# jontio/JAERO

Measured on NVIDIA H100. Metric: IQ Msamples/s (10.5k OQPSK demod + Viterbi), higher is better.
Workload: dtype f64

## Files before the change

jaero_b200/csrc/capi.cu:

```cuda
#include "../../include/jaero_b200.h"
#include "common.cuh"
#include "viterbi.cuh"
#include "demod.cuh"
#include "prefilter.cuh"
#include "pchannel.cuh"
#include "burst.cuh"
#include "rtchannel.cuh"
#include "cchannel.cuh"
#include "ddc.cuh"
#include "scan.cuh"
#include <cstring>
#include <complex>
#include <climits>
#include <cstdlib>
#include <initializer_list>
#include <new>
#include <numeric>
#include <vector>

namespace jb {
static thread_local std::string g_err;
void set_error(const std::string &m) { g_err = m; }
int cuda_fail(cudaError_t e, const char *what, const char *file, int line)
{
// ... 671 lines not shown
        b->slot_of.resize(cp);
        std::vector<int> ident(cp);
        for (size_t c = 0; c < cp; c++) { ident[c] = (int)c; b->slot_of[c] = (int)c; }
        JB_CUDA(cudaMemcpy(b->d_chan_of, ident.data(), cp * sizeof(int), cudaMemcpyHostToDevice));
        p.chan_of = b->d_chan_of;
        b->next_regroup = 34;
    }
    JB_CUDA(cudaMallocHost(&b->h_ints, (size_t)I_COUNT * cp * sizeof(int)));
    JB_CUDA(cudaMallocHost(&b->h_dbls, (size_t)D_COUNT * cp * sizeof(double)));
    JB_CUDA(cudaMallocHost(&b->h_soft_total, cp * sizeof(long long)));
    JB_CUDA(cudaMallocHost(&b->h_soft_stage, (size_t)n_channels * p.soft_cap * sizeof(int16_t)));
    guard.release();
    *out = b;
    return JAERO_OK;
}

void jaero_batch_destroy(jaero_batch *b)
{
    if (!b) return;
    cudaSetDevice(b->device);
    cudaStreamSynchronize(b->stream);
    if (b->copy_stream) { cudaStreamSynchronize(b->copy_stream); cudaStreamDestroy(b->copy_stream); }
    if (b->ev_stage_free) cudaEventDestroy(b->ev_stage_free);
    for (int k = 0; k < 8; k++) if (b->ev_slice[k]) cudaEventDestroy(b->ev_slice[k]);
    for (auto &e : b->ev_seg) { cudaEventDestroy(e.first); cudaEventDestroy(e.second); }
    for (auto &e : b->ev_cfe) { cudaEventDestroy(e.first); cudaEventDestroy(e.second); }
    release(b, {b->d_stage, b->d_x, b->d_ring_scratch}, {b->h_ints, b->h_dbls, b->h_soft_stage, b->h_soft_total, b->h_keys}, b->own_stream);
}
int jaero_batch_channels(const jaero_batch *b) { return b ? b->p.n_channels : 0; }
int64_t jaero_batch_launch_count(const jaero_batch *b) { return b ? b->launches : 0; }

int jaero_batch_set_stream(jaero_batch *b, void *cuda_stream)
{
    if (!b) { set_error("null handle"); return JAERO_E_ARG; }
    JB_CUDA(cudaSetDevice(b->device));
    JB_CUDA(cudaStreamSynchronize(b->stream));
    b->stream = cuda_stream ? (cudaStream_t)cuda_stream : b->own_stream;
    return JAERO_OK;
}
int jaero_batch_set_profiling(jaero_batch *b, int enabled)
{
    if (!b) { set_error("null handle"); return JAERO_E_ARG; }
    b->profiling = enabled != 0;
    return JAERO_OK;
}
int jaero_batch_get_profile(jaero_batch *b, double out[5])
{
    if (!b || !out) { set_error("null argument"); return JAERO_E_ARG; }
    JB_CUDA(cudaSetDevice(b->device));
    JB_CUDA(cudaStreamSynchronize(b->stream));
    double seg = 0, cfe = 0;
    for (auto &e : b->ev_seg) { float ms = 0; cudaEventElapsedTime(&ms, e.first, e.second); seg += ms; cudaEventDestroy(e.first); cudaEventDestroy(e.second); }
    for (auto &e : b->ev_cfe) { float ms = 0; cudaEventElapsedTime(&ms, e.first, e.second); cfe += ms; cudaEventDestroy(e.first); cudaEventDestroy(e.second); }
    out[0] = seg; out[1] = (double)b->ev_seg.size(); out[2] = cfe; out[3] = (double)b->ev_cfe.size(); out[4] = b->prof_samples;
    b->ev_seg.clear(); b->ev_cfe.clear(); b->prof_samples = 0;
    return JAERO_OK;
}
int jaero_batch_cfe_clusters(const jaero_batch *b) { return b ? b->cfe.clusters : 0; }

int jaero_batch_cfe_geometry(const jaero_batch *b, int32_t out[6])
{
    if (!b || !out) { set_error("jaero_batch_cfe_geometry: null argument"); return JAERO_E_ARG; }
    const CfePlan &c = b->cfe;
    out[0] = c.nfft; out[1] = b->p.bb_len; out[2] = c.lo; out[3] = c.hi; out[4] = c.expectedpeakbin; out[5] = c.clusters;
    return JAERO_OK;
}
int jaero_batch_probe_cfe(jaero_batch *b, const double *ring, int oldest, const int32_t *bigchange, int impl, int max_clusters,
                          int max_group, double *y_out, double *raw_est, double *emitted_est)
{
    if (!b || !ring) { set_error("jaero_batch_probe_cfe: null argument"); return JAERO_E_ARG; }
    DemodParams &p = b->p;
    const int C = p.n_channels, N = b->cfe.nfft;
    const size_t cp = p.cpad;
    if (oldest < 0 || oldest >= p.bb_len) { set_error("jaero_batch_probe_cfe: oldest outside the ring"); return JAERO_E_ARG; }
    if (impl < 0 || impl > 2 || max_clusters < 0 || max_group < 0) {
        set_error("jaero_batch_probe_cfe: bad impl / max_clusters / max_group"); return JAERO_E_ARG; }
    CfePlan plan = b->cfe;
    if (max_group > 0) plan.group = std::min(plan.group, max_group);
    JB_CUDA(cudaSetDevice(b->device));
    int clusters = b->cfe.clusters;
    if (impl == 1) clusters = 0;
    if (impl == 2) {
        clusters = (N == 16384) ? cfe_cluster_capacity() : 0;
        if (clusters <= 0) { set_error("jaero_batch_probe_cfe: the cluster estimator is not available for this batch / device"); return JAERO_E_STATE; }
    }
    if (clusters > 0 && max_clusters > 0) clusters = std::min(clusters, max_clusters);
    JB_CUDA(cudaStreamSynchronize(b->stream));
    const cudaStream_t s = b->stream;
    std::vector<int> em, zb;
    JB_CUDA(cudaMemcpyAsync(p.bb, ring, (size_t)C * p.bb_len * sizeof(double2), cudaMemcpyHostToDevice, s));
    if (bigchange) {
        em.resize(C); zb.resize(C);
        JB_CUDA(cudaMemcpyAsync(em.data(), p.I + (size_t)I_EMPTYING * cp, C * sizeof(int), cudaMemcpyDeviceToHost, s));
        JB_CUDA(cudaMemcpyAsync(zb.data(), p.I + (size_t)I_ZERO_BB * cp, C * sizeof(int), cudaMemcpyDeviceToHost, s));
        JB_CUDA(cudaStreamSynchronize(s));
        for (int c = 0; c < C; c++) if (bigchange[c]) { em[c] = 4; zb[c] = 1; }
        JB_CUDA(cudaMemcpyAsync(p.I + (size_t)I_EMPTYING * cp, em.data(), C * sizeof(int), cudaMemcpyHostToDevice, s));
        JB_CUDA(cudaMemcpyAsync(p.I + (size_t)I_ZERO_BB * cp, zb.data(), C * sizeof(int), cudaMemcpyHostToDevice, s));
    }
    if (clusters > 0 ? cfe_cluster_run(plan, p, oldest, std::min(clusters, C), s, &b->launches)
                     : cfe_run(plan, p, oldest, s, &b->launches)) return JAERO_E_CUDA;
    if (y_out) JB_CUDA(cudaMemcpyAsync(y_out, b->cfe.y, (size_t)C * N * sizeof(double), cudaMemcpyDeviceToHost, s));
    if (raw_est) JB_CUDA(cudaMemcpyAsync(raw_est, p.D + (size_t)D_CFE_EST * cp, C * sizeof(double), cudaMemcpyDeviceToHost, s));
    if (emitted_est) JB_CUDA(cudaMemcpyAsync(emitted_est, p.cfe_est_out, C * sizeof(double), cudaMemcpyDeviceToHost, s));
    JB_CUDA(cudaStreamSynchronize(s));
    return JAERO_OK;
}

int jaero_batch_sync(jaero_batch *b)
{
    if (!b) { set_error("null handle"); return JAERO_E_ARG; }
    JB_CUDA(cudaSetDevice(b->device));
    JB_CUDA(cudaStreamSynchronize(b->stream));
    return JAERO_OK;
}

int jaero_batch_write_device(jaero_batch *b, const int16_t *d_pcm, size_t n, size_t stride)
{
    if (!b || !d_pcm) { set_error("jaero_batch_write_device: null argument"); return JAERO_E_ARG; }
    if (n == 0) return JAERO_OK;
    if (stride < n || n > 0x7fffffff) { set_error("jaero_batch_write_device: bad stride / length"); return JAERO_E_ARG; }
    JB_CUDA(cudaSetDevice(b->device));
    const DemodParams &p = b->p;
    if ((((uintptr_t)d_pcm) & 15) || (stride & 7)) {
        const size_t C = p.n_channels, pitch = (n + 7) & ~(size_t)7;
        if (d_pcm == b->d_stage) { set_error("internal: staging buffer misaligned"); return JAERO_E_STATE; }
        if (grow(&b->d_stage, &b->stage_cap, C * pitch, b->stream)) return JAERO_E_CUDA;
        JB_CUDA(cudaMemcpy2DAsync(b->d_stage, pitch * sizeof(int16_t), d_pcm, stride * sizeof(int16_t), n * sizeof(int16_t), C,
                                  cudaMemcpyDeviceToDevice, b->stream));
        d_pcm = b->d_stage; stride = pitch;
    }
    if (b->pre_on) {
        while (b->next_slice < b->n_slices) { JB_CUDA(cudaStreamWaitEvent(b->stream, b->ev_slice[b->next_slice], 0)); b->next_slice++; }
        const size_t C = p.n_channels, xs = (n + 7) & ~(size_t)7;
        if (grow(&b->d_x, &b->x_cap, C * xs, b->stream)) return JAERO_E_CUDA;
        b->pre.x = b->d_x; b->pre.xstride = xs;
        b->p.xpre = b->d_x; b->p.xstride = xs;
        if (pre_down_launch(b->pre, d_pcm, stride, (int)n, b->stream)) return JAERO_E_CUDA;
        b->launches++;
        int i = 0;
        while (i < (int)n) {
            const int room = FIR_L - b->fir_fill;
            const int take = std::min(room, (int)n - i);
            if (fir_exchange_up_launch(b->pre, b->fir, i, i + take, b->fir_fill, b->stream)) return JAERO_E_CUDA;
            b->launches++;
            b->fir_fill += take; i += take;
            if (b->fir_fill == FIR_L) {
                if (fir_block_launch(b->fir, p.n_channels, b->fir_blocks == 0 ? 1 : 0, b->stream)) return JAERO_E_CUDA;
                b->launches++;
                b->fir_fill = 0; b->fir_blocks++;
            }
        }
    }
    peak_kernel<<<(p.n_channels + 3) / 4, 128, 0, b->stream>>>(p, d_pcm, stride, (int)n);
    JB_CUDA(cudaGetLastError());
    b->launches++;
    const int N = p.bbnfft, trig_every = p.cpu_reduce ? N : N / 4;
    SegmentArgs a;
    memset(&a, 0, sizeof a);
    a.new_write = 1;
    int seg_start = 0; bool resume = false;
    auto launch = [&](int i0, int i1, bool stop_after_a, int bb0, int cc0) -> int {
        a.sample0 = b->samples; a.i0 = i0; a.i1 = i1; a.skip_a_first = resume ? 1 : 0; a.stop_after_a = stop_after_a ? 1 : 0;
        a.apply_cfe = resume ? 1 : 0; a.bb_pos = bb0; a.coarse_counter = cc0;
        while (b->next_slice < b->n_slices && b->next_slice * b->slice_len < i1) {
            JB_CUDA(cudaStreamWaitEvent(b->stream, b->ev_slice[b->next_slice], 0));
            b->next_slice++;
        }
        cudaEvent_t e0 = 0, e1 = 0;
        if (b->profiling) { cudaEventCreate(&e0); cudaEventCreate(&e1); cudaEventRecord(e0, b->stream); }
        int r = (p.kind == JAERO_KIND_MSK) ? msk_pipe_launch(p, a, d_pcm, stride, b->stream)
                : (p.fb > 8400)            ? oqpsk_pipe_launch(p, a, d_pcm, stride, b->stream)
                                           : oqpsk_segment_launch(p, a, d_pcm, stride, b->stream);
        if (b->profiling) { cudaEventRecord(e1, b->stream); b->ev_seg.push_back({e0, e1}); b->prof_samples += (i1 - i0 - (stop_after_a ? 1 : 0)); }
        b->launches++;
        a.new_write = 0;
        return r;
    };
    int bb = b->bb_pos, cc = b->coarse_counter;
    int seg_bb = bb, seg_cc = cc;
    for (int i = 0; i < (int)n; i++) {
        bool trigger = false;
        if (cc >= p.Fs || !p.cpu_reduce) {
            bb++; if (bb >= N) bb = 0;
            if (bb % trig_every == 0) trigger = true;
        }
        if (trigger) {
            if (launch(seg_start, i + 1, true, seg_bb, seg_cc)) return JAERO_E_CUDA;
            b->samples += (i - seg_start);
            cudaEvent_t c0 = 0, c1 = 0;
            if (b->profiling) { cudaEventCreate(&c0); cudaEventCreate(&c1); cudaEventRecord(c0, b->stream); }
            if (b->cfe.clusters > 0 ? cfe_cluster_run(b->cfe, p, bb, std::min(b->cfe.clusters, p.n_channels), b->stream, &b->launches)
                                    : cfe_run(b->cfe, p, bb, b->stream, &b->launches)) return JAERO_E_CUDA;
            if (b->profiling) { cudaEventRecord(c1, b->stream); b->ev_cfe.push_back({c0, c1}); }
            b->epochs++;
            if (b->next_regroup >= 0 && b->epochs >= b->next_regroup) {
                b->next_regroup = b->epochs + (b->epochs < 64 ? 32 : REGROUP_EVERY);
                if (batch_regroup_by_phase(b, false)) return JAERO_E_CUDA;
            }
            cc = 0;
            seg_start = i; resume = true; seg_bb = bb; seg_cc = 0;
        }
        cc++;
    }
    if (launch(seg_start, (int)n, false, seg_bb, seg_cc)) return JAERO_E_CUDA;
    b->samples += ((int)n - seg_start);
    while (b->next_slice < b->n_slices) { JB_CUDA(cudaStreamWaitEvent(b->stream, b->ev_slice[b->next_slice], 0)); b->next_slice++; }
    b->n_slices = 0; b->next_slice = 0;
    b->bb_pos = bb; b->coarse_counter = cc;
    if (b->pre_on) {
        if (pre_finish_launch(b->pre, p.m2_freq_sum, (int)n, p.Fs, b->stream)) return JAERO_E_CUDA;
        b->launches++;
    }
    return JAERO_OK;
}

int jaero_batch_write(jaero_batch *b, const int16_t *pcm, size_t n, size_t stride)
{
    if (!b || !pcm) { set_error("jaero_batch_write: null argument"); return JAERO_E_ARG; }
    if (n == 0) return JAERO_OK;
    if (stride < n) { set_error("jaero_batch_write: channel_stride < n_samples"); return JAERO_E_ARG; }
    JB_CUDA(cudaSetDevice(b->device));
    const size_t C = b->p.n_channels;
    const size_t pitch = (n + 7) & ~(size_t)7;
    if (grow(&b->d_stage, &b->stage_cap, C * pitch, b->stream)) return JAERO_E_CUDA;
    if (n < 8192) {
        JB_CUDA(cudaMemcpy2DAsync(b->d_stage, pitch * sizeof(int16_t), pcm, stride * sizeof(int16_t), n * sizeof(int16_t), C,
                                  cudaMemcpyHostToDevice, b->stream));
        return jaero_batch_write_device(b, b->d_stage, n, pitch);
    }
    if (!b->copy_stream) {
        JB_CUDA(cudaStreamCreateWithFlags(&b->copy_stream, cudaStreamNonBlocking));
        JB_CUDA(cudaEventCreateWithFlags(&b->ev_stage_free, cudaEventDisableTiming));
        for (int k = 0; k < 8; k++) JB_CUDA(cudaEventCreateWithFlags(&b->ev_slice[k], cudaEventDisableTiming));
    }
    JB_CUDA(cudaEventRecord(b->ev_stage_free, b->stream));
    JB_CUDA(cudaStreamWaitEvent(b->copy_stream, b->ev_stage_free, 0));
    b->slice_len = (int)((((n + 7) / 8) + 7) & ~(size_t)7);
    b->n_slices = 0; b->next_slice = 0;
    for (size_t s0 = 0; s0 < n; s0 += (size_t)b->slice_len) {
        const size_t len = std::min((size_t)b->slice_len, n - s0);
        JB_CUDA(cudaMemcpy2DAsync(b->d_stage + s0, pitch * sizeof(int16_t), pcm + s0, stride * sizeof(int16_t), len * sizeof(int16_t), C,
                                  cudaMemcpyHostToDevice, b->copy_stream));
        JB_CUDA(cudaEventRecord(b->ev_slice[b->n_slices], b->copy_stream));
        b->n_slices++;
    }
    return jaero_batch_write_device(b, b->d_stage, n, pitch);
}

static int pull_ints(jaero_batch *b)
{
    const size_t cp = b->p.cpad;
    JB_CUDA(cudaMemcpyAsync(b->h_ints, b->p.I, (size_t)I_COUNT * cp * sizeof(int), cudaMemcpyDeviceToHost, b->stream));
    JB_CUDA(cudaStreamSynchronize(b->stream));
    return 0;
}

int jaero_batch_read_softbits(jaero_batch *b, int16_t *out, size_t cap, int32_t *counts)
{
    if (!b || !out || !counts) { set_error("jaero_batch_read_softbits: null argument"); return JAERO_E_ARG; }
    JB_CUDA(cudaSetDevice(b->device));
    return drain_softbits(b->p, b->p.I, I_COUNT, I_SOFT_COUNT, I_SOFT_OVERFLOW, b->h_ints, b->h_soft_stage, b->stream, out, cap, counts);
}
int jaero_batch_softbits_device(jaero_batch *b, const int16_t **d_soft, const int32_t **d_counts, size_t *ring_cap)
{
    if (!b || !d_soft || !d_counts || !ring_cap) { set_error("null argument"); return JAERO_E_ARG; }
    *d_soft = b->p.soft; *d_counts = b->p.I + (size_t)I_SOFT_COUNT * b->p.cpad; *ring_cap = (size_t)b->p.soft_cap;
    return JAERO_OK;
}
int jaero_batch_reset_softbits(jaero_batch *b)
{
    if (!b) { set_error("null handle"); return JAERO_E_ARG; }
    JB_CUDA(cudaSetDevice(b->device));
    return soft_reset(b->p, b->stream);
}
int jaero_batch_set_dcd(jaero_batch *b, int channel, int dcd)
{
    if (!b || channel >= b->p.n_channels) { set_error("jaero_batch_set_dcd: bad argument"); return JAERO_E_ARG; }
    JB_CUDA(cudaSetDevice(b->device));
    return launch_set_int(b->p.I + (size_t)I_DCD * b->p.cpad, b->p.n_channels, channel, dcd ? 1 : 0, b->stream);
}
int jaero_batch_set_center_freq(jaero_batch *b, int channel, double hz)
{
    if (!b || channel >= b->p.n_channels) { set_error("jaero_batch_set_center_freq: bad argument"); return JAERO_E_ARG; }
    JB_CUDA(cudaSetDevice(b->device));
    center_freq_kernel<<<(b->p.n_channels + 127) / 128, 128, 0, b->stream>>>(b->p, channel, hz);
    JB_CUDA(cudaGetLastError());
    return JAERO_OK;
}
int jaero_batch_set_afc(jaero_batch *b, int state)
{
    if (!b) { set_error("null handle"); return JAERO_E_ARG; }
    b->p.afc = state ? 1 : 0;
    return JAERO_OK;
}
int jaero_batch_set_sql(jaero_batch *b, int state)
{
    if (!b) { set_error("null handle"); return JAERO_E_ARG; }
    b->p.sql = state ? 1 : 0;
    return JAERO_OK;
}
int jaero_batch_wire_signal_status(jaero_batch *b, int enabled)
{
    if (!b) { set_error("null handle"); return JAERO_E_ARG; }
    b->p.wire_sigstat = enabled ? 1 : 0;
    return JAERO_OK;
}
int jaero_batch_regroup(jaero_batch *b, const int32_t *slot_of)
{
    if (!b) { set_error("null handle"); return JAERO_E_ARG; }
    if (!b->d_chan_of) return JAERO_OK;
    JB_CUDA(cudaSetDevice(b->device));
    if (!slot_of) return batch_regroup_by_phase(b, true) ? JAERO_E_CUDA : JAERO_OK;
    const int C = b->p.n_channels, cp = b->p.cpad;
    std::vector<int> v(cp), seen(C, 0);
    for (int c = 0; c < C; c++) { if (slot_of[c] < 0 || slot_of[c] >= C || seen[slot_of[c]]) { set_error("jaero_batch_regroup: not a permutation"); return JAERO_E_ARG; } seen[slot_of[c]] = 1; v[c] = slot_of[c]; }
    for (int c = C; c < cp; c++) v[c] = c;
    return batch_apply_seating(b, v) ? JAERO_E_CUDA : JAERO_OK;
}
int jaero_batch_set_cpu_reduce(jaero_batch *b, int state)
{
    if (!b) { set_error("null handle"); return JAERO_E_ARG; }
    b->p.cpu_reduce = state ? 1 : 0;
    return JAERO_OK;
}
int jaero_batch_get_status_all(jaero_batch *b, jaero_status *out)
{
    if (!b || !out) { set_error("null argument"); return JAERO_E_ARG; }
    JB_CUDA(cudaSetDevice(b->device));
    const size_t cp = b->p.cpad;
    JB_CUDA(cudaMemcpyAsync(b->h_dbls, b->p.D, (size_t)D_COUNT * cp * sizeof(double), cudaMemcpyDeviceToHost, b->stream));
    JB_CUDA(cudaMemcpyAsync(b->h_soft_total, b->p.soft_total, cp * sizeof(long long), cudaMemcpyDeviceToHost, b->stream));
    if (pull_ints(b)) return JAERO_E_CUDA;
    for (int ch = 0; ch < b->p.n_channels; ch++) {
        auto D = [&](int i) { return b->h_dbls[(size_t)i * cp + ch]; };
        auto I = [&](int i) { return b->h_ints[(size_t)i * cp + ch]; };
        jaero_status &s = out[ch];
        s.mixer2_freq = D(D_M2_FREQ); s.mixer2_wtptr = D(D_M2_PTR); s.center_freq = D(D_MC_FREQ);
        s.st_freq = D(D_ST_FREQ); s.st_wtptr = D(D_ST_PTR); s.agc = D(D_AGC_VAL); s.mse = D(D_MSE);
        s.ebno = D(D_EB_EBNO); s.marg = D(D_MARG_VAL); s.cfe_est = D(D_CFE_EST);
        s.n_sig_true = I(I_SIG_TRUE); s.n_sig_false = I(I_SIG_FALSE);
        s.center_wtptr = D(D_MC_PTR); s.st_ref_wtptr = D(D_SR_PTR);
        s.samples = b->samples; s.softbits = b->h_soft_total[ch] + I(I_SOFT_COUNT); s.dcd = I(I_DCD); s.reserved = 0;
        s.peak_volume = (double)I(I_PEAK) / 32768.0;
        s.scatter[0] = D(D_SCAT0_RE); s.scatter[1] = D(D_SCAT0_IM); s.scatter[2] = D(D_SCAT1_RE); s.scatter[3] = D(D_SCAT1_IM);
    }
    JB_CUDA(cudaMemsetAsync(b->p.I + (size_t)I_PEAK * cp, 0, cp * sizeof(int), b->stream));
    return JAERO_OK;
}
int jaero_batch_get_status(jaero_batch *b, int channel, jaero_status *out)
{
    if (!b || !out || channel < 0 || channel >= b->p.n_channels) { set_error("jaero_batch_get_status: bad argument"); return JAERO_E_ARG; }
    std::vector<jaero_status> all(b->p.n_channels);
    int r = jaero_batch_get_status_all(b, all.data());
    if (r) return r;
    *out = all[channel];
    return JAERO_OK;
}

}

// ... 1336 lines not shown
```

jaero_b200/csrc/cfe.cu:

```cuda
#include "demod_device.cuh"
#include "fft_device.cuh"
#include <cooperative_groups.h>
#include <cstring>

namespace jb {

static const int TILE = 16;
static const int MAXN = 128;
static const int CFE_THREADS = 256;

template <bool INV, int R>
__device__ __forceinline__ void stockham_pass(double2 (*s)[MAXN + 1], int n, int Ns, const double2 *__restrict__ tw, int tw_stride)
{
    stockham_pass<INV, R, TILE, MAXN + 1, CFE_THREADS>(s, n, Ns, tw, tw_stride);
}

template <bool INV>
__device__ __forceinline__ void tile_fft(double2 (*s)[MAXN + 1], int n, const double2 *__restrict__ tw, int tw_stride)
{
    stockham_pass<INV, 8>(s, n, 1, tw, tw_stride);
    if (n == 128) { stockham_pass<INV, 4>(s, n, 8, tw, tw_stride); stockham_pass<INV, 4>(s, n, 32, tw, tw_stride); }
    else if (n == 64) stockham_pass<INV, 8>(s, n, 8, tw, tw_stride);
    else stockham_pass<INV, 4>(s, n, 8, tw, tw_stride);
}

template <bool FUSED_INV_SQUARE>
__global__ void __launch_bounds__(CFE_THREADS)
cfe_col_kernel(CfePlan pl, const double2 *__restrict__ src, double2 *__restrict__ dst, size_t src_pitch, int rot, int ring_len, int ch0)
{
    __shared__ double2 s[TILE][MAXN + 1];
    const int ch = blockIdx.y;
    const int c0 = blockIdx.x * TILE;
    const int n1 = pl.n1, n2 = pl.n2, N = pl.nfft;
    const double2 *in = src + (size_t)(ch0 + ch) * src_pitch;
    double2 *out = dst + (size_t)ch * N;
    for (int e = threadIdx.x; e < n1 * TILE; e += CFE_THREADS) {
        const int r = e / TILE, cc = e - r * TILE;
        int n = n2 * r + c0 + cc;
        if (!FUSED_INV_SQUARE) { n += rot; if (n >= ring_len) n -= ring_len; }
        s[cc][r] = in[n];
    }
    __syncthreads();
    if (FUSED_INV_SQUARE) {
        tile_fft<true>(s, n1, pl.tw, N / n1);
        for (int e = threadIdx.x; e < n1 * TILE; e += CFE_THREADS) {
            const int cc = e / n1, r = e - cc * n1;
            const double2 x = s[cc][r];
            s[cc][r] = make_double2(x.x * x.x - x.y * x.y, x.x * x.y + x.y * x.x);
        }
        __syncthreads();
    }
    tile_fft<false>(s, n1, pl.tw, N / n1);
    for (int e = threadIdx.x; e < n1 * TILE; e += CFE_THREADS) {
        const int k1 = e / TILE, cc = e - k1 * TILE;
        const int c = c0 + cc;
        const double2 w = pl.tw[(c * k1) & (N - 1)];
        const double2 x = s[cc][k1];
        out[(size_t)k1 * n2 + c] = make_double2(x.x * w.x - x.y * w.y, x.x * w.y + x.y * w.x);
    }
}

__global__ void __launch_bounds__(CFE_THREADS)
cfe_row_mask_kernel(CfePlan pl, const double2 *__restrict__ src, double2 *__restrict__ dst)
{
    __shared__ double2 s[TILE][MAXN + 1];
    const int ch = blockIdx.y;
    const int r0 = blockIdx.x * TILE;
    const int n1 = pl.n1, n2 = pl.n2, N = pl.nfft;
    const double2 *in = src + (size_t)ch * N;
    double2 *out = dst + (size_t)ch * N;
    for (int e = threadIdx.x; e < n2 * TILE; e += CFE_THREADS) {
        const int rr = e / n2, c = e - rr * n2;
        s[rr][c] = in[(size_t)(r0 + rr) * n2 + c];
    }
    __syncthreads();
    tile_fft<false>(s, n2, pl.tw, N / n2);
    for (int e = threadIdx.x; e < n2 * TILE; e += CFE_THREADS) {
        const int rr = e / n2, k2 = e - rr * n2;
        const int k = (r0 + rr) + n1 * k2;
        double2 x = s[rr][k2];
        if (!pl.is8400) { if (k >= pl.startbin && k <= pl.stopbin) x = make_double2(0.0, 0.0); }
        else { const double w = pl.window[k]; x = make_double2(x.x * w, x.y * w); }
        s[rr][k2] = x;
    }
    __syncthreads();
    tile_fft<true>(s, n2, pl.tw, N / n2);
    for (int e = threadIdx.x; e < n2 * TILE; e += CFE_THREADS) {
        const int rr = e / n2, c = e - rr * n2;
        const int k1 = r0 + rr;
        double2 w = pl.tw[(c * k1) & (N - 1)];
        w.y = -w.y;
        const double2 x = s[rr][c];
        out[(size_t)k1 * n2 + c] = make_double2(x.x * w.x - x.y * w.y, x.x * w.y + x.y * w.x);
    }
}

__global__ void __launch_bounds__(CFE_THREADS)
cfe_row_logmag_kernel(CfePlan pl, DemodParams p, const double2 *__restrict__ src, int ch0)
{
    __shared__ double2 s[TILE][MAXN + 1];
    const int ch = blockIdx.y;
    const int r0 = blockIdx.x * TILE;
    const int n1 = pl.n1, n2 = pl.n2, N = pl.nfft;
    const double2 *in = src + (size_t)ch * N;
    double *y = pl.y + (size_t)(ch0 + ch) * N;
    const bool bigchange = p.I[(size_t)I_ZERO_BB * p.cpad + ch0 + ch] != 0;
    for (int e = threadIdx.x; e < n2 * TILE; e += CFE_THREADS) {
        const int rr = e / n2, c = e - rr * n2;
        s[rr][c] = in[(size_t)(r0 + rr) * n2 + c];
    }
    __syncthreads();
    tile_fft<false>(s, n2, pl.tw, N / n2);
    for (int e = threadIdx.x; e < n2 * TILE; e += CFE_THREADS) {
        const int k2 = e / TILE, rr = e - k2 * TILE;
        const int k1 = r0 + rr;
        const int k2s = (k2 + (n2 >> 1)) & (n2 - 1);
        const int i = k1 + n1 * k2s;
        const double2 x = s[rr][k2];
        const double mag = hypot(x.x, x.y);
        const double yo = bigchange ? 20.0 : y[i];
        y[i] = yo * 0.9 + 0.1 * 10 * log10(fmax(mag, 1.0));
    }
}

__global__ void __launch_bounds__(128)
cfe_search_kernel(CfePlan pl, DemodParams p)
{
    const int lane = threadIdx.x & 31;
    const int ch = blockIdx.x * (blockDim.x >> 5) + (threadIdx.x >> 5);
    if (ch >= p.n_channels) return;
    const double *y = pl.y + (size_t)ch * pl.nfft;
    const int N = pl.nfft, epb = pl.expectedpeakbin;
    double best = 0.0; int besti = 0x7fffffff;
    int i0 = pl.lo;
    if (pl.lo - epb - 1 >= 0 && pl.hi + epb + 1 < N) {
        for (; i0 + 128 <= pl.hi; i0 += 128) {
            double a[4][3], c[4][3];
#pragma unroll
            for (int u = 0; u < 4; u++) {
                const int i = i0 + lane + 32 * u;
#pragma unroll
                for (int j = -1; j <= 1; j++) { a[u][j + 1] = y[i - epb - j]; c[u][j + 1] = y[i + epb + j]; }
            }
#pragma unroll
            for (int u = 0; u < 4; u++) {
                double val = 0;
#pragma unroll
                for (int j = 0; j < 3; j++) val += (a[u][j] + c[u][j]);
                if (val > best) { best = val; besti = i0 + lane + 32 * u; }
            }
        }
    }
    for (int i = i0 + lane; i < pl.hi; i += 32) {
        if ((i < 0) || (i >= N)) continue;
        double val = 0;
        for (int j = -1; j <= 1; j++) {
            if (((i - epb - j) < 0) || ((i + epb + j) >= N)) continue;
            val += (y[i - epb - j] + y[i + epb + j]);
        }
        if (val > best) { best = val; besti = i; }
    }
    for (int off = 16; off > 0; off >>= 1) {
        const double ob = __shfl_xor_sync(0xffffffffu, best, off);
        const int oi = __shfl_xor_sync(0xffffffffu, besti, off);
        if (ob > best || (ob == best && oi < besti)) { best = ob; besti = oi; }
    }
    if (lane == 0) {
        const int zmaxloc = (best > 0.0) ? besti : N / 2;
        const double est = -((double)(zmaxloc - N / 2)) * pl.hzperbin * 0.5;
        p.D[(size_t)D_CFE_EST * p.cpad + ch] = est;
        int &emptying = p.I[(size_t)I_EMPTYING * p.cpad + ch];
        if (emptying <= 0) p.cfe_est_out[ch] = est;
        else { emptying--; p.cfe_est_out[ch] = 0.0; }
        p.I[(size_t)I_ZERO_BB * p.cpad + ch] = 0;
    }
}

namespace cgx = cooperative_groups;

static const int CC_CL = 8, CC_T = 128, CC_SEQ = 16, CC_RS = 143;
static const int CC_BUF = CC_SEQ * CC_RS * 16;
static const int CC_TW2 = 128, CC_TW3 = 152;
static const int CC_SM_TOTAL = 2 * CC_BUF + (128 + 24 + 32) * 16;

__device__ __forceinline__ int cc_ph(int e) { return e + (e >> 3); }

__device__ __forceinline__ double log10_ge1(double x)
{
    const double Lg1 = 6.666666666666735130e-01, Lg2 = 3.999999999940941908e-01, Lg3 = 2.857142874366239149e-01, Lg4 = 2.222219843214978396e-01,
                 Lg5 = 1.818357216161805012e-01, Lg6 = 1.531383769920937332e-01, Lg7 = 1.479819860511658591e-01;
    const double ivln10 = 4.34294481903251816668e-01, log10_2hi = 3.01029995663611771306e-01, log10_2lo = 3.69423907715893078616e-13;
    int hi = __double2hiint(x);
    const int lo = __double2loint(x);
    int k = (hi >> 20) - 1023;
    hi &= 0x000fffff;
    const int i = (hi + 0x95f64) & 0x100000;
    hi |= (i ^ 0x3ff00000);
    k += (i >> 20);
    const double f = __hiloint2double(hi, lo) - 1.0;
    const double s = div_fast(f, 2.0 + f);
    const double z = s * s, w = z * z;
    const double t1 = w * (Lg2 + w * (Lg4 + w * Lg6));
    const double t2 = z * (Lg1 + w * (Lg3 + w * (Lg5 + w * Lg7)));
    const double hfsq = 0.5 * f * f;
    const double lg = f - (hfsq - s * (hfsq + (t2 + t1)));
    const double dk = (double)k;
    return (dk * log10_2lo + ivln10 * lg) + dk * log10_2hi;
}

__device__ __forceinline__ void cc_load16(const double2 *row, int k, double2 (&x)[16])
{
#pragma unroll
    for (int p = 0; p < 16; p++) x[p] = row[cc_ph(k + 8 * p)];
}

__device__ __forceinline__ void cc_store16(double2 *row, int k, const double2 (&x)[16])
{
#pragma unroll
    for (int p = 0; p < 16; p++) row[cc_ph(k + 8 * p)] = x[p];
}

template <bool INV>
__device__ __forceinline__ void cc_pass23(double2 (&x)[16], int k, const double2 *__restrict__ tws)
{
    auto radix4 = [](double2 &v0, double2 &v1, double2 &v2, double2 &v3, double2 w1, double2 w2, double2 w3) {
        if (INV) { w1.y = -w1.y; w2.y = -w2.y; w3.y = -w3.y; }
        v1 = c_mul(v1, w1); v2 = c_mul(v2, w2); v3 = c_mul(v3, w3);
        dft4<INV>(v0, v1, v2, v3);
    };
    double2 y[16];
    {
        const double2 w1 = tws[CC_TW2 + k], w2 = tws[CC_TW2 + 8 + k], w3 = tws[CC_TW2 + 16 + k];
#pragma unroll
        for (int m = 0; m < 4; m++) {
            double2 v0 = x[m], v1 = x[m + 4], v2 = x[m + 8], v3 = x[m + 12];
            radix4(v0, v1, v2, v3, w1, w2, w3);
            y[4 * m] = v0; y[4 * m + 1] = v1; y[4 * m + 2] = v2; y[4 * m + 3] = v3;
        }
    }
#pragma unroll
    for (int u = 0; u < 4; u++) {
        const int l = k + 8 * u;
        double2 v0 = y[u], v1 = y[u + 4], v2 = y[u + 8], v3 = y[u + 12];
        radix4(v0, v1, v2, v3, tws[l], tws[CC_TW3 + l], tws[3 * l]);
        x[u] = v0; x[u + 4] = v1; x[u + 8] = v2; x[u + 12] = v3;
    }
}

template <bool INV>
__device__ __forceinline__ void cc_pass1_store(const double2 (&x)[16], double2 *row, int k)
{
    double2 a[8], b[8];
#pragma unroll
    for (int t = 0; t < 8; t++) { a[t] = x[2 * t]; b[t] = x[2 * t + 1]; }
    dft8<INV>(a);
    dft8<INV>(b);
    __syncwarp();
#pragma unroll
    for (int t = 0; t < 8; t++) { row[cc_ph(8 * k + t)] = a[t]; row[cc_ph(8 * k + 64 + t)] = b[t]; }
    __syncwarp();
}

__global__ void __launch_bounds__(CC_T, 2)
cfe_cluster_kernel(CfePlan pl, DemodParams p, int oldest)
{
    extern __shared__ __align__(128) unsigned char cc_smem[];
    double2 *bufA = reinterpret_cast<double2 *>(cc_smem);
    double2 *bufB = reinterpret_cast<double2 *>(cc_smem + CC_BUF);
    double2 *tws = reinterpret_cast<double2 *>(cc_smem + 2 * CC_BUF);
    cgx::cluster_group cluster = cgx::this_cluster();
    const int q = (int)cluster.block_rank();
    const int n_clusters = gridDim.x / CC_CL, cid = blockIdx.x / CC_CL;
    const int N = 16384, ring_len = p.bb_len;
    const double2 *__restrict__ twN = pl.tw;
    for (int t = threadIdx.x; t < 128 + 24 + 32; t += CC_T) {
        if (t < 128) tws[t] = twN[t * (N / 128)];
        else if (t < 128 + 24) { const int e = t - 128, m = e >> 3, k = e & 7; tws[CC_TW2 + e] = twN[(4 * (m + 1) * k) * (N / 128)]; }
        else { const int l = t - 152; tws[CC_TW3 + l] = twN[(2 * l) * (N / 128)]; }
    }
    __syncthreads();
    bool arrived = false;
    cluster.sync();
    const int f = threadIdx.x >> 3, k = threadIdx.x & 7;
    double2 *const rowA = bufA + f * CC_RS, *const rowB = bufB + f * CC_RS;
    for (int ch = cid; ch < p.n_channels; ch += n_clusters) {
        double2 x[16];
        double2 colv[2][8];
        {
            const double2 *ring = p.bb + (size_t)ch * ring_len;
            const int cc = threadIdx.x & 15, r0i = threadIdx.x >> 4;
#pragma unroll
            for (int h = 0; h < 2; h++)
#pragma unroll
                for (int i = 0; i < 8; i++) {
                    int n = oldest + 128 * (r0i + 8 * h + 16 * i) + 16 * q + cc;
                    if (n >= ring_len) n -= ring_len;
                    if (n >= ring_len) n -= ring_len;
                    colv[h][i] = ring[n];
                }
        }
        dft8<false>(colv[0]);
        dft8<false>(colv[1]);
        if (arrived) { cluster.barrier_wait(); arrived = false; }
        {
            const int cc = threadIdx.x & 15, r0i = threadIdx.x >> 4;
#pragma unroll
            for (int h = 0; h < 2; h++)
#pragma unroll
                for (int i = 0; i < 8; i++) bufA[cc * CC_RS + cc_ph(8 * (r0i + 8 * h) + i)] = colv[h][i];
        }
        __syncthreads();
        cc_load16(rowA, k, x);
        cc_pass23<false>(x, k, tws);
        cc_store16(rowA, k, x);
        double2 tw8[2][8];
        {
            const int kk = threadIdx.x & 15, cc = threadIdx.x >> 4;
#pragma unroll
            for (int h = 0; h < 2; h++)
#pragma unroll
                for (int s = 0; s < 8; s++) tw8[h][s] = __ldg(&twN[((16 * s + cc + 8 * h) * (16 * q + kk)) & (N - 1)]);
        }
        cluster.sync();
        {
            const int kk = threadIdx.x & 15;
#pragma unroll
            for (int h = 0; h < 2; h++) {
                const int cc = (threadIdx.x >> 4) + 8 * h;
                double2 v[8];
#pragma unroll
                for (int s = 0; s < 8; s++) v[s] = c_mul(cluster.map_shared_rank(bufA, s)[cc * CC_RS + cc_ph(16 * q + kk)], tw8[h][s]);
                dft8<false>(v);
#pragma unroll
                for (int s = 0; s < 8; s++) bufB[kk * CC_RS + cc_ph(8 * cc + s)] = v[s];
            }
        }
        __syncthreads();
        cc_load16(rowB, k, x);
        cc_pass23<false>(x, k, tws);
#pragma unroll
        for (int e = 0; e < 16; e++) {
            const int bin = (16 * q + f) + 128 * (k + 8 * e);
            if (!pl.is8400) { if (bin >= pl.startbin && bin <= pl.stopbin) x[e] = make_double2(0.0, 0.0); }
            else {
                const double w = pl.window[bin];
                x[e] = make_double2(__dmul_rn(x[e].x, w), __dmul_rn(x[e].y, w));
            }
        }
        cc_pass1_store<true>(x, rowB, k);
        cc_load16(rowB, k, x);
        cc_pass23<true>(x, k, tws);
        cc_store16(rowB, k, x);
        {
            const int cc = threadIdx.x & 15, kk = threadIdx.x >> 4;
#pragma unroll
            for (int h = 0; h < 2; h++)
#pragma unroll
                for (int s = 0; s < 8; s++) tw8[h][s] = __ldg(&twN[((16 * q + cc) * (16 * s + kk + 8 * h)) & (N - 1)]);
        }
        cluster.sync();
        {
            const int cc = threadIdx.x & 15;
#pragma unroll
            for (int h = 0; h < 2; h++) {
                const int kk = (threadIdx.x >> 4) + 8 * h;
                double2 v[8];
#pragma unroll
                for (int s = 0; s < 8; s++) {
                    double2 w = tw8[h][s]; w.y = -w.y;
                    v[s] = c_mul(cluster.map_shared_rank(bufB, s)[kk * CC_RS + cc_ph(16 * q + cc)], w);
                }
                dft8<true>(v);
#pragma unroll
                for (int s = 0; s < 8; s++) bufA[cc * CC_RS + cc_ph(8 * kk + s)] = v[s];
            }
        }
        __syncthreads();
        cc_load16(rowA, k, x);
        cc_pass23<true>(x, k, tws);
#pragma unroll
        for (int e = 0; e < 16; e++) x[e] = make_double2(x[e].x * x[e].x - x[e].y * x[e].y, x[e].x * x[e].y + x[e].y * x[e].x);
        cc_pass1_store<false>(x, rowA, k);
        cc_load16(rowA, k, x);
        cc_pass23<false>(x, k, tws);
        cc_store16(rowA, k, x);
        {
            const int kk = threadIdx.x & 15, cc = threadIdx.x >> 4;
#pragma unroll
            for (int h = 0; h < 2; h++)
#pragma unroll
                for (int s = 0; s < 8; s++) tw8[h][s] = __ldg(&twN[((16 * s + cc + 8 * h) * (16 * q + kk)) & (N - 1)]);
        }
        cluster.sync();
        {
            const int kk = threadIdx.x & 15;
#pragma unroll
            for (int h = 0; h < 2; h++) {
                const int cc = (threadIdx.x >> 4) + 8 * h;
                double2 v[8];
#pragma unroll
                for (int s = 0; s < 8; s++) v[s] = c_mul(cluster.map_shared_rank(bufA, s)[cc * CC_RS + cc_ph(16 * q + kk)], tw8[h][s]);
                dft8<false>(v);
#pragma unroll
                for (int s = 0; s < 8; s++) bufB[kk * CC_RS + cc_ph(8 * cc + s)] = v[s];
            }
        }
        cluster.barrier_arrive();
        arrived = true;
        __syncthreads();
        {
            double *y = pl.y + (size_t)ch * N;
            const bool bigchange = p.I[(size_t)I_ZERO_BB * p.cpad + ch] != 0;
            const int need_lo = pl.lo - pl.expectedpeakbin - 1, need_hi = pl.hi + pl.expectedpeakbin + 1;
            double yo[16];
#pragma unroll
            for (int e = 0; e < 16; e++) {
                const int i_sh = (16 * q + f) + 128 * ((k + 8 * e + 64) & 127);
                yo[e] = (bigchange || i_sh < need_lo || i_sh > need_hi) ? 20.0 : y[i_sh];
            }
            cc_load16(rowB, k, x);
            cc_pass23<false>(x, k, tws);
#pragma unroll
            for (int e = 0; e < 16; e++) {
                const int i_sh = (16 * q + f) + 128 * ((k + 8 * e + 64) & 127);
                if (i_sh < need_lo || i_sh > need_hi) continue;
                y[i_sh] = yo[e] * 0.9 + 0.1 * 5 * log10_ge1(fmax(x[e].x * x[e].x + x[e].y * x[e].y, 1.0));
            }
        }
        __syncthreads();
    }
    if (arrived) cluster.barrier_wait();
    cluster.sync();
}

int cfe_cluster_run(const CfePlan &pl, const DemodParams &p, int oldest, int n_clusters, cudaStream_t s, long long *launches)
{
    cudaLaunchConfig_t cfg;
    memset(&cfg, 0, sizeof cfg);
    cfg.gridDim = dim3((unsigned)(n_clusters * CC_CL)); cfg.blockDim = dim3(CC_T); cfg.dynamicSmemBytes = CC_SM_TOTAL; cfg.stream = s;
    cudaLaunchAttribute at; at.id = cudaLaunchAttributeClusterDimension; at.val.clusterDim.x = CC_CL; at.val.clusterDim.y = 1; at.val.clusterDim.z = 1;
    cfg.attrs = &at; cfg.numAttrs = 1;
    JB_CUDA(cudaLaunchKernelEx(&cfg, cfe_cluster_kernel, pl, p, oldest));
    cfe_search_kernel<<<(p.n_channels + 3) / 4, 128, 0, s>>>(pl, p);
    JB_CUDA(cudaGetLastError());
    *launches += 2;
    return 0;
}
int cfe_cluster_capacity()
{
    if (cudaFuncSetAttribute(cfe_cluster_kernel, cudaFuncAttributeMaxDynamicSharedMemorySize, CC_SM_TOTAL) != cudaSuccess) { cudaGetLastError(); return 0; }
    cudaLaunchConfig_t cfg;
    memset(&cfg, 0, sizeof cfg);
    cfg.gridDim = dim3(CC_CL * 64); cfg.blockDim = dim3(CC_T); cfg.dynamicSmemBytes = CC_SM_TOTAL;
    cudaLaunchAttribute at; at.id = cudaLaunchAttributeClusterDimension; at.val.clusterDim.x = CC_CL; at.val.clusterDim.y = 1; at.val.clusterDim.z = 1;
    cfg.attrs = &at; cfg.numAttrs = 1;
    int n = 0;
    if (cudaOccupancyMaxActiveClusters(&n, cfe_cluster_kernel, &cfg) != cudaSuccess) { cudaGetLastError(); return 0; }
    return n;
}

int cfe_run(const CfePlan &pl, const DemodParams &p, int oldest, cudaStream_t s, long long *launches)
{
    const int C = p.n_channels;
    for (int ch0 = 0; ch0 < C; ch0 += pl.group) {
        const int g = (C - ch0 < pl.group) ? C - ch0 : pl.group;
        dim3 gc(pl.n2 / TILE, g), gr(pl.n1 / TILE, g);
        cfe_col_kernel<false><<<gc, CFE_THREADS, 0, s>>>(pl, p.bb, pl.work_a, (size_t)p.bb_len, oldest, p.bb_len, ch0);
        cfe_row_mask_kernel<<<gr, CFE_THREADS, 0, s>>>(pl, pl.work_a, pl.work_b);
        cfe_col_kernel<true><<<gc, CFE_THREADS, 0, s>>>(pl, pl.work_b, pl.work_a, (size_t)pl.nfft, 0, pl.nfft, 0);
        cfe_row_logmag_kernel<<<gr, CFE_THREADS, 0, s>>>(pl, p, pl.work_a, ch0);
        *launches += 4;
    }
    cfe_search_kernel<<<(C + 3) / 4, 128, 0, s>>>(pl, p);
    *launches += 1;
    JB_CUDA(cudaGetLastError());
    return 0;
}

}
```

Before: 2665.

## Split CFE peak search across eight warps per channel and move peak_kernel launch

The CFE search kernel now gives each channel a whole block of eight warps instead of one warp, splitting the bin range into 128-aligned spans. Per-warp maxima are merged through shared memory with the same tie-break rule, and blocks run channels in reverse order. Separately, peak_kernel is launched after the segment pipeline instead of before it, presumably so it no longer delays the latency-critical demod chain. The cost is an extra block-level barrier, and the reordering matters only if peak_kernel's outputs are not needed by the segments.

```diff
diff --git a/jaero_b200/csrc/capi.cu b/jaero_b200/csrc/capi.cu
--- a/jaero_b200/csrc/capi.cu
+++ b/jaero_b200/csrc/capi.cu
@@ -847,9 +847,6 @@
             }
         }
     }
-    peak_kernel<<<(p.n_channels + 3) / 4, 128, 0, b->stream>>>(p, d_pcm, stride, (int)n);
-    JB_CUDA(cudaGetLastError());
-    b->launches++;
     const int N = p.bbnfft, trig_every = p.cpu_reduce ? N : N / 4;
     SegmentArgs a;
     memset(&a, 0, sizeof a);
@@ -902,6 +899,9 @@
     b->samples += ((int)n - seg_start);
     while (b->next_slice < b->n_slices) { JB_CUDA(cudaStreamWaitEvent(b->stream, b->ev_slice[b->next_slice], 0)); b->next_slice++; }
     b->n_slices = 0; b->next_slice = 0;
+    peak_kernel<<<(p.n_channels + 3) / 4, 128, 0, b->stream>>>(p, d_pcm, stride, (int)n);
+    JB_CUDA(cudaGetLastError());
+    b->launches++;
     b->bb_pos = bb; b->coarse_counter = cc;
     if (b->pre_on) {
         if (pre_finish_launch(b->pre, p.m2_freq_sum, (int)n, p.Fs, b->stream)) return JAERO_E_CUDA;
diff --git a/jaero_b200/csrc/cfe.cu b/jaero_b200/csrc/cfe.cu
--- a/jaero_b200/csrc/cfe.cu
+++ b/jaero_b200/csrc/cfe.cu
@@ -123,18 +123,22 @@
     }
 }
 
-__global__ void __launch_bounds__(128)
+static const int CFE_SEARCH_WARPS = 8;
+__global__ void __launch_bounds__(32 * CFE_SEARCH_WARPS)
 cfe_search_kernel(CfePlan pl, DemodParams p)
 {
-    const int lane = threadIdx.x & 31;
-    const int ch = blockIdx.x * (blockDim.x >> 5) + (threadIdx.x >> 5);
-    if (ch >= p.n_channels) return;
+    __shared__ double s_best[CFE_SEARCH_WARPS];
+    __shared__ int s_besti[CFE_SEARCH_WARPS];
+    const int lane = threadIdx.x & 31, warp = threadIdx.x >> 5;
+    const int ch = p.n_channels - 1 - (int)blockIdx.x;
     const double *y = pl.y + (size_t)ch * pl.nfft;
     const int N = pl.nfft, epb = pl.expectedpeakbin;
+    const int span = ((pl.hi - pl.lo + CFE_SEARCH_WARPS - 1) / CFE_SEARCH_WARPS + 127) & ~127;
+    const int lo = pl.lo + warp * span, hi = min(pl.hi, lo + span);
     double best = 0.0; int besti = 0x7fffffff;
-    int i0 = pl.lo;
+    int i0 = lo;
     if (pl.lo - epb - 1 >= 0 && pl.hi + epb + 1 < N) {
-        for (; i0 + 128 <= pl.hi; i0 += 128) {
+        for (; i0 + 128 <= hi; i0 += 128) {
             double a[4][3], c[4][3];
 #pragma unroll
             for (int u = 0; u < 4; u++) {
@@ -151,7 +155,7 @@
             }
         }
     }
-    for (int i = i0 + lane; i < pl.hi; i += 32) {
+    for (int i = i0 + lane; i < hi; i += 32) {
         if ((i < 0) || (i >= N)) continue;
         double val = 0;
         for (int j = -1; j <= 1; j++) {
@@ -160,12 +164,12 @@
         }
         if (val > best) { best = val; besti = i; }
     }
-    for (int off = 16; off > 0; off >>= 1) {
-        const double ob = __shfl_xor_sync(0xffffffffu, best, off);
-        const int oi = __shfl_xor_sync(0xffffffffu, besti, off);
-        if (ob > best || (ob == best && oi < besti)) { best = ob; besti = oi; }
-    }
-    if (lane == 0) {
+    auto merge = [&](double ob, int oi) { if (ob > best || (ob == best && oi < besti)) { best = ob; besti = oi; } };
+    for (int off = 16; off > 0; off >>= 1) merge(__shfl_xor_sync(0xffffffffu, best, off), __shfl_xor_sync(0xffffffffu, besti, off));
+    if (lane == 0) { s_best[warp] = best; s_besti[warp] = besti; }
+    __syncthreads();
+    if (threadIdx.x == 0) {
+        for (int w = 1; w < CFE_SEARCH_WARPS; w++) merge(s_best[w], s_besti[w]);
         const int zmaxloc = (best > 0.0) ? besti : N / 2;
         const double est = -((double)(zmaxloc - N / 2)) * pl.hzperbin * 0.5;
         p.D[(size_t)D_CFE_EST * p.cpad + ch] = est;
@@ -441,7 +445,7 @@
     cudaLaunchAttribute at; at.id = cudaLaunchAttributeClusterDimension; at.val.clusterDim.x = CC_CL; at.val.clusterDim.y = 1; at.val.clusterDim.z = 1;
     cfg.attrs = &at; cfg.numAttrs = 1;
     JB_CUDA(cudaLaunchKernelEx(&cfg, cfe_cluster_kernel, pl, p, oldest));
-    cfe_search_kernel<<<(p.n_channels + 3) / 4, 128, 0, s>>>(pl, p);
+    cfe_search_kernel<<<p.n_channels, 32 * CFE_SEARCH_WARPS, 0, s>>>(pl, p);
     JB_CUDA(cudaGetLastError());
     *launches += 2;
     return 0;
@@ -471,7 +475,7 @@
         cfe_row_logmag_kernel<<<gr, CFE_THREADS, 0, s>>>(pl, p, pl.work_a, ch0);
         *launches += 4;
     }
-    cfe_search_kernel<<<(C + 3) / 4, 128, 0, s>>>(pl, p);
+    cfe_search_kernel<<<C, 32 * CFE_SEARCH_WARPS, 0, s>>>(pl, p);
     *launches += 1;
     JB_CUDA(cudaGetLastError());
     return 0;
```

After: 2690 (median of 6 runs). About the same (+0.9%).
